# llliuqingyu/RSPL-SLAM

Measured on AMD Instinct MI355X. Metric: stereo frames/sec SuperPoint+SuperGlue+localBA @752x480 (all-keyframe: 2xSP, 2xSG, 1 BA per frame), higher is better.
Workload: dtype fp16 MFMA with fp32 accumulation for SuperPoint/SuperGlue (the reference's TensorRT kFP16 engines), fp32 Sinkhorn/decode, fp64 BA

## Files before the change

rspl-slam_amd/csrc/ba.cpp:

```cpp
#include <immintrin.h>

#include <algorithm>
#include <chrono>
#include <cmath>
#include <cstdlib>
#include <cstring>
#include <limits>
#include <numeric>
#include <string>
#include <type_traits>
#include <memory>
#include <vector>
#include <condition_variable>
#include <deque>
#include <mutex>
#include <thread>

#include "ba_kernels.hpp"
#include "common.hpp"
#include "ba_stage.hpp"
#include "se3_host.hpp"

using namespace rspl;

// ... 364 lines not shown
  Ss = S;
  view_bank(b->bank[1], Ls, Ss);
}

void accept_swap(rspl_ba* b, ba::Problem& P, ba::Lin& Lr, ba::Sys& S, bool lin) {
  std::swap(P.T, P.Tn);
  std::swap(P.X, P.Xn);
  std::swap(P.L, P.Ln);
  if (!lin) return;
  std::swap(b->bank[0], b->bank[1]);
  view_bank(b->bank[0], Lr, S);
}

void arm_prof(rspl_ba* b, const ba::Active& A, ba::Sys& S) {
  if (!b->prof || b->prof_nb[0]) return;
  S.prof = b->prof;
  b->prof_A = A;
  b->prof_nb[0] = ba::chunk_count(A);
  b->prof_nb[1] = ba::update_errors_blocks(A) + A.n_lblk;
  b->prof_nb[2] = ba::update_errors_blocks(A);
  b->prof_nb[3] = A.nchk;
  b->prof_nb[4] = A.K;
}

struct SpecSetup {
  ba::Active A2{};
  uint8_t* level = nullptr;
  int iters2 = 0;
  bool queued = false;
  bool extra = false;
  bool topped_up = false;
};

struct SpecFinish {
  bool on = false;
  ba::Lin L{};
  int E = 0;
  const int* gmap = nullptr;
  uint8_t* inl = nullptr;
  double *Th = nullptr, *Xh = nullptr, *Lh = nullptr;
  unsigned long long q = 0;
};

void preupload_next(rspl_ba* b);

struct DevLmArgs {
  uint8_t* cls_level = nullptr;
  bool build_pp = false;
  SpecFinish* fin = nullptr;
  SpecSetup* nxt = nullptr;
  bool setup_done = false;
};

int optimize_dev(rspl_ba* b, ba::Problem& P, ba::Lin& Lr, ba::Sys& S, const ba::Active& A, int iters,
                 double* chi2_out, int* done_out, const DevLmArgs& d) {
  hipStream_t st = b->stream;
  uint8_t* const cls_level = d.cls_level;
  SpecFinish* const fin = d.fin;
  SpecSetup* const nxt = d.nxt;
  S.lm = b->lmctl;
  S.lm_slot = 0;
  static const bool trace = getenv("RSPL_BA_LMTRACE") != nullptr;
  if (trace && !b->lm_trace) {
    RSPL_HIP(hipMalloc((void**)&b->lm_trace, sizeof(double) * 8 * 64));
    RSPL_HIP(hipMemset(b->lm_trace, 0, sizeof(double) * 8 * 64));
  }
  S.lm_trace = trace ? b->lm_trace + (iters == 10 ? 0 : 8 * 32) : nullptr;
  if (d.setup_done) {
  } else {
    int rg;
    if ((rg = grow_device(b, b->pdg, b->pdg_cap, (size_t)ba::setup_pdg_len(A), (size_t)1 << 14, 4u))) return rg;
    ba::Sys Su = S;
    Su.prof = b->prof && !b->prof_nb[0] && !cls_level ? b->prof : nullptr;
    RSPL_HIP(ba::setup_dev(P, Lr, A, Su, cls_level, cls_level ? const_cast<uint8_t*>(A.lm_act) : nullptr, iters,
                           d.build_pp ? b->pp_cnt : nullptr, b->pp_off, b->pp_buf, b->pdg, st));
  }
  unsigned long long q = b->seq;
  const unsigned long long q_first = b->seq + 1;
  ba::Lin Ls;
  ba::Sys Ss;
  bank_views(b, Lr, S, Ls, Ss);
  int queued = 0;
  const int kev0 = b->kev_used;
  auto enqueue = [&](int n) -> int {
    for (int k = 0; k < n; k++, queued++) {
      q = ++b->seq;
      ba::Spec sp{Ls, Ss};
      if (queued == 3) arm_prof(b, A, S);
      S.lm_slot = queued & 1;
      S.lm_post = k == n - 1;
      hipEvent_t* ev = nullptr;
      if (b->ktime_on) {
        if ((size_t)3 * (b->kev_used + 1) > b->kev.size()) {
          for (int i = 0; i < 3; i++) {
            hipEvent_t e;
            RSPL_HIP(hipEventCreate(&e));
            b->kev.push_back(e);
          }
          b->grew |= 8;
        }
        ev = &b->kev[3 * (size_t)b->kev_used++];
      }
      const hipError_t e = ba::trial_dev(P, Lr, A, S, q, st, sp, ev);
      S.prof = nullptr;
      if (e != hipSuccess) {
        set_error("BA trial launch failed: %s", hipGetErrorString(e));
        return RSPL_E_DEVICE;
      }
    }
    return RSPL_OK;
  };
  int rc;
  unsigned long long q_last = 0;
  auto enqueue_batch = [&](int n) -> int {
    int r;
    if ((r = enqueue(n))) return r;
    q_last = b->seq;
    if (fin) {
      ba::Sys Sf = S;
      Sf.lm = b->lmctl;
      Sf.lm_slot = queued & 1;
      Sf.prof = nullptr;
      fin->q = ++b->seq;
      fin->on = true;
      RSPL_HIP(ba::finish(P, fin->L, fin->E, fin->gmap, fin->inl, fin->Th, fin->Xh, fin->Lh, Sf, fin->q, st));
    }
    return RSPL_OK;
  };
  if ((rc = enqueue_batch(iters))) return rc;
  if (fin) preupload_next(b);
  auto queue_spec_setup = [&]() -> int {
    if (!nxt || (size_t)ba::setup_pdg_len(nxt->A2) > b->pdg_cap) return RSPL_OK;
    ba::Sys S2 = S;
    S2.lm = b->lmctl;
    S2.lm_slot = 0;
    S2.prof = nullptr;
    S2.lm_trace = nullptr;
    RSPL_HIP(ba::setup_dev(P, Lr, nxt->A2, S2, nxt->level, const_cast<uint8_t*>(nxt->A2.lm_act), nxt->iters2,
                           nullptr, b->pp_off, b->pp_buf, b->pdg, st, queued & 1, &Ls, &Ss));
    nxt->queued = true;
    nxt->extra = false;
    return RSPL_OK;
  };
  if ((rc = queue_spec_setup())) return rc;
  double v[4];
  for (;;) {
    if ((rc = spin_mail(b, "the LM trials", [&] {
          const unsigned long long s1 = __atomic_load_n(&b->mail->seq, __ATOMIC_ACQUIRE);
          if (s1 >= q_first && s1 <= q_last) {
            volatile const double* mv = b->mail->v;
            for (int k = 0; k < 4; k++) v[k] = mv[k];
            __atomic_thread_fence(__ATOMIC_ACQUIRE);
            return __atomic_load_n(&b->mail->vseq, __ATOMIC_ACQUIRE) == s1 && (s1 == q_last || v[3] != 0.0);
          }
          if (fin && s1 == fin->q) {
            volatile const double* mv = b->mail->v;
            for (int k = 0; k < 4; k++) v[k] = mv[k];
            __atomic_thread_fence(__ATOMIC_ACQUIRE);
            const unsigned long long vs = __atomic_load_n(&b->mail->vseq, __ATOMIC_ACQUIRE);
            return vs >= q_first && vs <= q_last && v[3] != 0.0;
          }
          return false;
        })))
      return rc;
    if (v[3] != 0.0) {
      if (b->ktime_on) {
        unsigned long long s1 = __atomic_load_n(&b->mail->seq, __ATOMIC_ACQUIRE);
        for (unsigned long long t = q_first; t <= s1 && t <= q_last; t++) b->kev_eval.push_back(kev0 + (int)(t - q_first));
      }
      break;
    }
    if (nxt) nxt->extra = nxt->topped_up = true;
    if ((rc = enqueue_batch(std::max(1, iters - (int)v[1])))) return rc;
    if ((rc = queue_spec_setup())) return rc;
  }
  S.lm = nullptr;
  if (v[2] != 0.0) accept_swap(b, P, Lr, S, true);
  *chi2_out = v[0];
  *done_out = (int)v[1];
  return RSPL_OK;
}

bool dev_lm(const rspl_ba* b, const ba::Active& A, int iters) {
  return b->allreduce == nullptr && iters > 0 && ba::fast_path(A.K);
}

int optimize_host(rspl_ba* b, ba::Problem& P, ba::Lin& Lr, ba::Sys& S, const ba::Active& A, int iters,
                  double* chi2_out, int* done_out) {
  hipStream_t st = b->stream;
  double v[4];
  int rc;
  const bool sh = b->allreduce != nullptr;
  const int n6 = 6 * A.K;
  double* so = b->red + n6 + b->nranks;
  unsigned long long q = ++b->seq;
  RSPL_HIP(ba::compute_errors(P, Lr, A, S, q, st));
  if (sh) {
    if (iters > 0) {
      RSPL_HIP(ba::linearize(P, Lr, A, S, true, st));
      RSPL_HIP(ba::shard_fold(A, S, b->red, b->rank, b->nranks, st));
      if ((rc = allreduce(b, b->red, ba::shard_red_len(A.K, b->nranks)))) return rc;
      RSPL_HIP(ba::shard_post(S, b->red, n6, b->nranks, 0, 0, q, st));
    } else {
      if ((rc = allreduce(b, so, 3))) return rc;
      RSPL_HIP(ba::shard_post(S, b->red, n6, b->nranks, 1, 0, q, st));
    }
  } else if (iters > 0) {
    RSPL_HIP(ba::linearize(P, Lr, A, S, true, st));
    q = ++b->seq;
// ... 699 lines not shown
    A.lmsub = cp.lmsub;
    ba::set_update_geometry(A);
  }
  A.n_line_edges = n_line_local;
  A.ltab = reinterpret_cast<const int4*>(cb + cl.ltab);
  A.n_lblk = n_lblk;
  A.K = K;
  A.nL = nL;
  A.robust = 1;
  A.pp_off = b->pp_off;
  A.pp = b->pp_buf;
  const bool pp_fused = dev_lm(b, A, pr->iterations_first);
  if (!pp_fused) RSPL_HIP(ba::build_pairs(A, b->pp_cnt, b->pp_off, b->pp_buf, st));
  tm.mark("pairs");
  SpecSetup nxt;
  nxt.A2 = A;
  nxt.A2.robust = 0;
  nxt.A2.elevel = level;
  nxt.A2.lm_act = b->lm_act2;
  nxt.level = level;
  nxt.iters2 = pr->iterations_second;
  const bool spec_setup = pp_fused && !sh && !b->ktime_on && dev_lm(b, nxt.A2, pr->iterations_second);
  DevLmArgs d1;
  d1.build_pp = pp_fused;
  d1.nxt = spec_setup ? &nxt : nullptr;
  if ((rc = optimize(b, P, Lr, S, A, pr->iterations_first, &res->chi2_first, &res->iterations_done_first, d1)))
    return rc;
  tm.mark("opt1");
  tr[5] = mono_s();
  uint8_t* inl_h = reinterpret_cast<uint8_t*>(b->stage_dev[c.slot] + dl.inl);
  double* T_h = reinterpret_cast<double*>(b->stage_dev[c.slot] + dl.T);
  double* X_h = reinterpret_cast<double*>(b->stage_dev[c.slot] + dl.X);
  double* L_h = reinterpret_cast<double*>(b->stage_dev[c.slot] + dl.L);
  SpecFinish fin;
  {
    A.robust = 0;
    A.elevel = level;
    A.lm_act = b->lm_act2;
    const bool fused = dev_lm(b, A, pr->iterations_second);
    if (!fused) {
      RSPL_HIP(ba::classify(P, Lr, E, level, nullptr, 0, st));
      RSPL_HIP(ba::landmark_active(A, level, b->lm_act2, st));
    }
    const bool spec_fin = fused && !sh && !b->ktime_on;
    if (spec_fin) {
      fin.L = Lr;
      fin.E = E;
      fin.gmap = reinterpret_cast<const int*>(cb + cl.gmap);
      fin.inl = inl_h;
      fin.Th = T_h;
      fin.Xh = X_h;
      fin.Lh = L_h;
    }
    DevLmArgs d2;
    d2.cls_level = fused ? level : nullptr;
    d2.fin = spec_fin ? &fin : nullptr;
    d2.setup_done = nxt.queued && !nxt.extra;
    if ((rc = optimize(b, P, Lr, S, A, pr->iterations_second, &res->chi2_second, &res->iterations_done_second, d2)))
      return rc;
    tm.mark("opt2");
    tr[6] = mono_s();
    tr[9] = (double)((unsigned)tr[9] | (nxt.queued && !nxt.extra ? 16u : 0u) | (nxt.topped_up ? 32u : 0u));
  }
  const unsigned long long q = fin.on ? fin.q : ++b->seq;
  if (fin.on) {
  } else if (sh) {
    const size_t glen = 3 * (size_t)nq + 6 * (size_t)nl + Eg;
    if ((rc = grow_device(b, b->gbuf, b->gcap, glen, (size_t)1024, 0u))) return rc;
    RSPL_HIP(hipMemsetAsync(b->gbuf, 0, sizeof(double) * glen, st));
    RSPL_HIP(ba::shard_gather(P, Lr, E, reinterpret_cast<const int*>(cb + cl.gmap), b->rank, b->nranks, b->gbuf, st));
    if (glen && (rc = allreduce(b, b->gbuf, glen))) return rc;
    RSPL_HIP(ba::shard_finish(P, Eg, b->gbuf, inl_h, T_h, X_h, L_h, S, q, st));
  } else {
    RSPL_HIP(ba::finish(P, Lr, E, reinterpret_cast<const int*>(cb + cl.gmap), inl_h, T_h, X_h, L_h, S, q, st));
  }
  if ((rc = wait_mail(b, q, nullptr))) return rc;
  if (b->ktime_on) {
    for (int i : b->kev_eval) {
      float a = 0.f, c = 0.f;
      if (hipEventElapsedTime(&a, b->kev[3 * (size_t)i], b->kev[3 * (size_t)i + 1]) == hipSuccess &&
          hipEventElapsedTime(&c, b->kev[3 * (size_t)i + 1], b->kev[3 * (size_t)i + 2]) == hipSuccess) {
        b->kt_ms[0] += a;
        b->kt_ms[1] += c;
        b->kt_n[0]++;
        b->kt_n[1]++;
      }
    }
  }
  if (b->prof && b->prof_nb[0]) report_prof(b);
  tr[9] = (double)((unsigned)tr[9] | b->grew);
  if (b->lm_trace) {
    std::vector<double> h(8 * 64);
    if (hipMemcpy(h.data(), b->lm_trace, sizeof(double) * h.size(), hipMemcpyDeviceToHost) == hipSuccess)
      for (int k = 0; k < 64; k++)
        if (h[8 * k] != 0.0)
          fprintf(stderr, "lmtrace phase %d trial %d chi2 %.17g scale %.6g fail %g lambda %.6g chi0 %.17g cur %g it %g q %g\n",
                  k / 32, k % 32, h[8 * k], h[8 * k + 1], h[8 * k + 2], h[8 * k + 3], h[8 * k + 4], h[8 * k + 5],
                  h[8 * k + 6], h[8 * k + 7]);
    (void)hipMemset(b->lm_trace, 0, sizeof(double) * h.size());
  }
  if (nq) memcpy(res->points, b->stage[c.slot] + dl.X, sizeof(double) * 3 * nq);
  if (nl) memcpy(res->lines, b->stage[c.slot] + dl.L, sizeof(double) * 6 * nl);
  const double* Tout = reinterpret_cast<const double*>(b->stage[c.slot] + dl.T);
  uint8_t* outs[4] = {res->mono_inlier, res->stereo_inlier, res->mono_line_inlier, res->stereo_line_inlier};
  int e = 0;
  for (int t = 0; t < 4; t++) {
    if (outs[t]) memcpy(outs[t], b->stage[c.slot] + dl.inl + e, ne[t]);
    e += ne[t];
  }
// ... 40 lines not shown
```

rspl-slam_amd/csrc/ba_first.hip:

```cpp
#include <hip/hip_runtime.h>

#include <algorithm>
#include <cstdint>

#include "ba_kernels.hpp"
#include "ba_linearize.hpp"

namespace rspl {
namespace ba {

__global__ __launch_bounds__(256) void post_kernel(Sys S, int K, int npd, unsigned long long seq) {
  __shared__ double part[4][64];
  if (npd > 0) {
    const int lane = threadIdx.x & 63, pt = threadIdx.x >> 6, nq6 = 6 * K;
    double mx = 0;
    for (int q0 = 0; q0 < nq6; q0 += 64) {
      const int q = q0 + lane;
      double sacc = 0;
      if (q < nq6) {
        const int pa = q / 6, i = q - 6 * pa;
        const double* src = S.partial2 + (size_t)pa * npd * 6 + i;
        for (int b = pt; b < npd; b += 4) sacc += src[(size_t)b * 6];
      }
      part[pt][lane] = sacc;
// ... 455 lines not shown
  if (g >= A.nL) return;
  uint8_t on = 0;
  for (int k = A.lm_off[g]; k < A.lm_off[g + 1]; k++) on |= level[(k)] == 0;
  lm_act[g] = on;
}

__device__ __forceinline__ bool edge_inlier(const Problem& P, const Lin& L, int e) {
  double chi2;
  bool depth_ok;
  edge_status(P, L, e, chi2, depth_ok);
  return chi2 <= pick4(P.th, P.etype[e]) && depth_ok;
}
__device__ __forceinline__ void classify_edge(const Problem& P, const Lin& L, int e, uint8_t* level, uint8_t* inlier,
                                              int final_pass) {
  if (final_pass) {
    inlier[e] = edge_inlier(P, L, e) ? 1 : 0;
    return;
  }
  double chi2;
  bool depth_ok;
  edge_status(P, L, e, chi2, depth_ok);
  if (chi2 > pick4(P.th, P.etype[e]) || !depth_ok) level[e] = 1;
}

__global__ __launch_bounds__(256) void classify_kernel(Problem P, Lin L, int E, uint8_t* level, uint8_t* inlier,
                                                       int final_pass) {
  const int e = blockIdx.x * blockDim.x + threadIdx.x;
  if (e < E) classify_edge(P, L, e, level, inlier, final_pass);
}

__global__ __launch_bounds__(256) void finish_kernel(Problem P, Lin L, int E, const int* gmap, uint8_t* inl, double* Th,
                                                     double* Xh, double* Lh, Sys S, unsigned long long seq) {
  __shared__ int last;
  if (S.lm) {
    const LmCtrl* c = S.lm + S.lm_slot;
    if (!c->stop) return;
    if (c->cur) bank_state(P);
  }
  const int i = blockIdx.x * blockDim.x + threadIdx.x;
  if (i < E) inl[gmap[i]] = edge_inlier(P, L, i) ? 1 : 0;
  if (i < 8 * P.np) Th[i] = P.T[i];
  if (i < 3 * P.nq) Xh[i] = P.X[i];
  if (i < 6 * P.nl) Lh[i] = P.L[i];
  __threadfence_system();
  __syncthreads();
  if (threadIdx.x == 0) {
    const unsigned tk = __hip_atomic_fetch_add(S.counter, 1u, __ATOMIC_ACQ_REL, __HIP_MEMORY_SCOPE_AGENT);
    last = tk == gridDim.x - 1;
  }
  __syncthreads();
  if (!last || threadIdx.x != 0) return;
  __hip_atomic_store(S.counter, 0u, __ATOMIC_RELAXED, __HIP_MEMORY_SCOPE_AGENT);
  __hip_atomic_store(&S.mail->seq, seq, __ATOMIC_RELEASE, __HIP_MEMORY_SCOPE_SYSTEM);
}

__global__ __launch_bounds__(256) void shard_fold_kernel(Sys S, double* red, int K, int npd, int rank, int nranks) {
  const int n6 = 6 * K;
  for (int q = threadIdx.x; q < n6; q += 256) {
    double acc = 0;
    if (npd > 0) {
      const int pa = q / 6, i = q - 6 * pa;
      const double* src = S.partial2 + (size_t)pa * npd * 6 + i;
      for (int b = 0; b < npd; b++) acc += src[(size_t)b * 6];
    }
    red[q] = acc;
  }
  for (int r = threadIdx.x; r < nranks; r += 256) red[n6 + r] = r == rank ? S.out[2] : 0.0;
}

__global__ void shard_post_kernel(Sys S, const double* red, int n6, int nranks, int mode, int add_pose_scale,
                                  unsigned long long seq) {
// ... 152 lines not shown
```

rspl-slam_amd/csrc/ba_kernels.hpp:

```cpp
#pragma once
#include <hip/hip_runtime.h>

#include <cstdint>

namespace rspl {
namespace ba {

struct Problem {
  const double* cams;
  double* T;
  double* X;
  double* L;
  double* Tn;
  double* Xn;
  double* Ln;
  int np, nq, nl;
  int ncam;
  const int8_t* etype;
  const int* epose;
  const int* elm;
  const int* ecam;
  const double* eobs;
  int Ep;
  double delta[4];
// ... 131 lines not shown
  double* chunk;
  double* pairfin;
  unsigned* pair_ctr;
  unsigned* solve_ctr;
  double* partial;
  double* partial2;
  double* out;
  int* fail;
  unsigned* counter;
  unsigned* lm_ctr;
  Mail* mail;
  double* shard_out;
  int pose_scale;
  unsigned long long* prof;
  LmCtrl* lm;
  double* lm_trace;
  int lm_slot;
  int lm_post;
};
constexpr int kProfPc = 16, kProfUe = kProfPc + 4 * 4096, kProfX = kProfUe + 4 * 4096, kProfLen = kProfX + 8;

constexpr int kLmChunk = 256;
constexpr int kLineBlk = 8;

hipError_t compute_errors(const Problem& P, const Lin& L, const Active& A, Sys& S, unsigned long long seq,
                          hipStream_t s);
hipError_t linearize(const Problem& P, const Lin& L, const Active& A, const Sys& S, bool with_maxdiag,
                     hipStream_t s);
hipError_t post(Sys& S, unsigned long long seq, hipStream_t s, const Active* A = nullptr);
hipError_t setup_dev(const Problem& P, const Lin& L, const Active& A, Sys& S, uint8_t* level, uint8_t* lm_act2,
                     int lm_iters, int* pp_cnt, int* pp_off, int4* pp, double* pdg, hipStream_t s, int gate = -1,
                     const Lin* Ls = nullptr, const Sys* Ss = nullptr);
int setup_pdg_len(const Active& A);
struct Spec {
  Lin Ls;
  Sys Ss;
};
hipError_t trial_host_large(const Problem& P, const Lin& L, const Active& A, Sys& S, double lambda,
                            unsigned long long seq, hipStream_t s);
hipError_t trial_dev(const Problem& P, const Lin& L, const Active& A, Sys& S, unsigned long long seq, hipStream_t s,
                     const Spec& spec, hipEvent_t* ev = nullptr);
hipError_t build_pairs(const Active& A, int* pp_cnt, int* pp_off, int4* pp, hipStream_t s);
hipError_t landmark_active(const Active& A, const uint8_t* level, uint8_t* lm_act, hipStream_t s);
hipError_t classify(const Problem& P, const Lin& L, int E, uint8_t* level, uint8_t* inlier, int final_pass,
                    hipStream_t s);
hipError_t finish(const Problem& P, const Lin& L, int E, const int* gmap, uint8_t* inl, double* Th, double* Xh,
                  double* Lh, Sys& S, unsigned long long seq, hipStream_t s);
hipError_t trial_chunks(const Problem& P, const Lin& L, const Active& A, Sys& S, double lambda, hipStream_t s);
hipError_t trial_solve(const Problem& P, const Lin& L, const Active& A, Sys& S, double lambda, hipStream_t s);
hipError_t shard_fold(const Active& A, Sys& S, double* red, int rank, int nranks, hipStream_t s);
hipError_t shard_post(Sys& S, const double* red, int n6, int nranks, int mode, int add_pose_scale,
                      unsigned long long seq, hipStream_t s);
hipError_t shard_gather(const Problem& P, const Lin& L, int E, const int* gmap, int rank, int nranks, double* G,
                        hipStream_t s);
hipError_t shard_finish(const Problem& P, int E_global, const double* G, uint8_t* inl, double* Th, double* Xh,
                        double* Lh, Sys& S, unsigned long long seq, hipStream_t s);
int shard_red_len(int K, int nranks);
bool fast_path(int K);
bool wave_path(int K);
int update_blocks(const Problem& P);
int errors_blocks(int Ea);
int update_errors_blocks(const Active& A);
void set_update_geometry(Active& A);

}
}
```

rspl-slam_amd/csrc/ba_linearize.hpp:

```cpp
#pragma once
#include "ba_device.hpp"
#include "wave_reduce.hpp"

namespace rspl {
namespace ba {

__device__ __forceinline__ double edge_weight_of(const Problem& P, const Active& A, const double* er, int t) {
  double w = einfo(t);
  if (A.robust) {
    double chi2 = 0;
    for (int k = 0; k < edim(t); k++) chi2 += er[k] * er[k];
    chi2 *= einfo(t);
    double r0, r1;
    huber(chi2, pick4(P.delta, t), r0, r1);
    w *= r1;
  }
  return w;
}

__device__ __forceinline__ void point_jac_R(int t, const double (&R)[9], const double* tt, const double* cam,
                                            const double* Xg, double (&Jp)[3][6], double (&Jl)[3][3]) {
  const double fx = cam[0], fy = cam[1], bf = cam[4];
  double Xc[3];
  mat3_vec(R, Xg, Xc);
// ... 201 lines not shown
    H[8] += lambda;
    const bool ok = small_inv<3>(H, Di);
#pragma unroll
    for (int i = 0; i < 4; i++)
#pragma unroll
      for (int j = 0; j < 4; j++) D[i * 4 + j] = (i < 3 && j < 3) ? Di[i * 3 + j] : 0.0;
    return ok;
  }
  double H[16];
#pragma unroll
  for (int i = 0; i < 16; i++) H[i] = Hll[i];
#pragma unroll
  for (int i = 0; i < 4; i++) H[i * 5] += lambda;
  return small_inv<4>(H, D);
}

__device__ __forceinline__ void cand_pose(const Problem& P, const Active& A, const double* x, int i, bool failed,
                                          double (&o)[8]) {
  const int a = A.pidx[i];
#pragma unroll
  for (int k = 0; k < 8; k++) o[k] = P.T[8 * i + k];
  if (a < 0 || failed) return;
  double xp[6];
#pragma unroll
  for (int k = 0; k < 6; k++) xp[k] = x[6 * a + k];
  const SE3 r = se3_mul(se3_exp(xp), load_T(o));
#pragma unroll
  for (int k = 0; k < 4; k++) o[k] = r.q[k];
#pragma unroll
  for (int k = 0; k < 3; k++) o[4 + k] = r.t[k];
  o[7] = 0;
}

__device__ __forceinline__ void edge_status(const Problem& P, const Lin& L, int e, double& chi2, bool& depth_ok) {
  const int t = P.etype[e];
  chi2 = 0;
  for (int k = 0; k < edim(t); k++) chi2 += L.err[4 * e + k] * L.err[4 * e + k];
  chi2 *= einfo(t);
  depth_ok = true;
  if (t < 2) {
    const SE3 T = load_T(P.T + 8 * P.epose[e]);
    double R[9], Xc[3];
    q_to_R(T.q, R);
    mat3_vec(R, P.X + 3 * P.elm[e], Xc);
    depth_ok = Xc[2] + T.t[2] > 0.0;
  }
}
constexpr int kLinPlain = 0, kLinSpec = 1, kLinSetup = 2;
__device__ __forceinline__ bool edge_outlier(const Problem& P, const Lin& L, int e) {
  double chi2;
  bool depth_ok;
  edge_status(P, L, e, chi2, depth_ok);
  return chi2 > pick4(P.th, P.etype[e]) || !depth_ok;
}
__device__ __forceinline__ bool line_active(const Problem& P, const Lin& L, const Active& A, int g, bool cls) {
  if (!cls) return A.lm_act[g] != 0;
  for (int k = A.lm_off[g]; k < A.lm_off[g + 1]; k++)
    if (!edge_outlier(P, L, k)) return true;
  return false;
}
template <int MODE>
__device__ __forceinline__ void lin_lines(const Problem& P, const Lin& L, const Active& A, const Sys& S, int blk,
                                          bool maxd, const Lin* Lc = nullptr, const Sys* Sc = nullptr,
                                          double lambda = 0.0, bool failed = false,
                                          unsigned long long* stamp = nullptr, bool cls = false,
                                          double* chi_out = nullptr, double* pdg = nullptr, int pd_nb = 0,
                                          int pd_b = 0) {
  constexpr bool SPEC = MODE == kLinSpec, SETUP = MODE == kLinSetup, OWN_ERR = SPEC || SETUP;
  __shared__ double ev[kLineBlk][20][4];
  __shared__ double J[kLineBlk][4 * 6 + 4 * 4];
  __shared__ double Lsh[kLineBlk][6];
  __shared__ double es[kLineBlk][4];
  __shared__ int einfo_s[kLineBlk][4];
  __shared__ double cv[kLineBlk][20];
  __shared__ double Tsh[kLineBlk][8];
  const int tid = threadIdx.x, wv = tid >> 6, lane = tid & 63;
  const int4 tb = A.ltab[blk];
  const int p0 = tb.x, cnt = tb.y & 0xff, gb = tb.z, ge = tb.w;
  const bool split = (tb.y >> 8) != 0;
// ... 354 lines not shown
```

rspl-slam_amd/csrc/ba_trial.hip:

```cpp
#include <hip/hip_runtime.h>

#include <cfloat>
#include <cstdint>

#include "ba_kernels.hpp"
#include "ba_launch.hpp"
#include "ba_linearize.hpp"

namespace rspl {
namespace ba {

__device__ int lm_decide(const LmCtrl* c, LmCtrl* n, double chi2, double scale, double fail) {
  const bool ok = fail == 0.0;
  const double tempChi = ok ? chi2 : DBL_MAX;
  double rho = c->chi - tempChi;
  rho /= ok ? scale + 1e-3 : 1.0;
  double lambda = c->lambda, ni = c->ni;
  int qmax = c->qmax, it = c->it;
  bool brk = false;
  *n = *c;
  if (rho > 0 && isfinite(tempChi) && ok) {
    double alpha = 1. - cube(2 * rho - 1);
    alpha = fmin(alpha, 2. / 3.);
    lambda *= fmax(1. / 3., alpha);
// ... 124 lines not shown
          const double* xp = S.x + 6 * max(as[u], 0);
#pragma unroll
          for (int j = 0; j < 4; j++) {
            double s = 0;
#pragma unroll
            for (int r = 0; r < 6; r++) s += B[r * 4 + j] * xp[r];
            c[j] -= as[u] >= 0 ? s : 0.0;
          }
        }
      }
      double D[16];
      if (!lm_dinv(S.Hll + 16 * g, point, lambda, D)) atomicOr(S.fail, 1);
#pragma unroll
      for (int r = 0; r < 4; r++) xl[r] = D[r * 4] * c[0] + D[r * 4 + 1] * c[1] + D[r * 4 + 2] * c[2] + D[r * 4 + 3] * c[3];
#pragma unroll
      for (int k = 0; k < 4; k++) sc += xl[k] * (lambda * xl[k] + S.bl[4 * g + k]);
    }
    if (point) {
      for (int k = 0; k < 3; k++) P.Xn[3 * g + k] = P.X[3 * g + k] + xl[k];
    } else {
      const int l = g - P.nq;
      double Lv[6];
      for (int k = 0; k < 6; k++) Lv[k] = P.L[6 * l + k];
      if (upd) line_oplus(Lv, xl);
      for (int k = 0; k < 6; k++) P.Ln[6 * l + k] = Lv[k];
    }
  }
  const double s = block_sum256(sc, red);
  if (threadIdx.x == 0) S.partial2[blockIdx.x] = s;
}

template <bool SPEC>
__global__ __launch_bounds__(256) void update_errors_kernel(Problem P, Lin L, Active A, Sys S, double lambda,
                                                            unsigned long long seq, Lin Ls, Sys Ss, int nbu) {
  __shared__ double red[4 * 2];
  __shared__ int last;
  const bool stamp = threadIdx.x == 0 && blockIdx.x < 4096;
  if (stamp) prof_stamp(S, kProfUe + 4 * blockIdx.x);
  bool spec = SPEC;
  if (SPEC && (int)blockIdx.x >= nbu) {
    if (S.lm) {
      LmView v;
      if (!lm_view(S, v)) return;
      lambda = v.lambda;
      spec = v.spec;
      if (v.cur) {
        bank_state(P);
        bank_lin(L, Ls, S, Ss);
      }
    }
    if (!spec) return;
    lin_lines<kLinSpec>(P, Ls, A, Ss, blockIdx.x - nbu, false, &L, &S, lambda, *S.fail != 0,
                    S.prof ? S.prof + kProfUe + 4 * blockIdx.x + 1 : nullptr);
    if (stamp) prof_stamp(S, kProfUe + 4 * blockIdx.x + 3);
    return;
  }
  if (!SPEC) nbu = gridDim.x;
  __shared__ double sT[64 * 8], scam[16 * 5], sx[6 * 32];
  const int tid = threadIdx.x;
  int ub = blockIdx.x;
  if (SPEC && A.ue_bpr > 0) {
    const int b = blockIdx.x, x = b & 7, sl = b >> 3, r = sl / A.ue_bpr, lb = 8 * r + x;
    constexpr int per = 64 * kUeWaves / kGroup;
    ub = lb < A.nchk ? lb * A.ue_bpr + (sl - r * A.ue_bpr) : (A.nL + per - 1) / per + 1;
  }
  const int t = ub * (64 * kUeWaves) + tid, g = t / kGroup, j = t % kGroup;
  const bool in = tid < 64 * kUeWaves && g < A.nL;
  const bool point = g < P.nq;
  int k0 = 0, k1 = 0;
  bool act = false;
  double dl[16], blg[4], lm[6] = {0, 0, 0, 0, 0, 0};
  double dl2[16], blg2[4], lm2[6] = {0, 0, 0, 0, 0, 0};
// ... 7 lines not shown
    act = A.lm_act[g] != 0;
#pragma unroll
    for (int q = 0; q < 16; q++) {
      dl[q] = point && q >= 9 ? 0.0 : S.Hll[16 * g + q];
      dl2[q] = point && q >= 9 ? 0.0 : Ss.Hll[16 * g + q];
    }
#pragma unroll
    for (int q = 0; q < 4; q++) {
      blg[q] = S.bl[4 * g + q];
      blg2[q] = Ss.bl[4 * g + q];
    }
    if (point) {
#pragma unroll
      for (int q = 0; q < 3; q++) {
        lm[q] = P.X[3 * g + q];
        lm2[q] = P.Xn[3 * g + q];
      }
    } else {
#pragma unroll
      for (int q = 0; q < 6; q++) {
        lm[q] = P.L[6 * (g - P.nq) + q];
        lm2[q] = P.Ln[6 * (g - P.nq) + q];
      }
    }
  }
  if (S.lm) {
    LmView v;
    if (!lm_view(S, v)) {
      if (blockIdx.x == 0 && threadIdx.x == 0) S.lm[S.lm_slot ^ 1] = S.lm[S.lm_slot];
      return;
    }
    lambda = v.lambda;
    spec = SPEC && v.spec;
    if (v.cur) {
      bank_state(P);
      bank_lin(L, Ls, S, Ss);
#pragma unroll
      for (int q = 0; q < 16; q++) dl[q] = dl2[q];
#pragma unroll
      for (int q = 0; q < 4; q++) blg[q] = blg2[q];
#pragma unroll
      for (int q = 0; q < 6; q++) lm[q] = lm2[q];
    }
  }
  const bool failed = *S.fail != 0;
  for (int q = tid; q < 5 * P.ncam; q += 256) scam[q] = P.cams[q];
  for (int q = tid; q < 6 * A.K; q += 256) sx[q] = S.x[q];
  const int kf = k0 + j;
  const bool has = in && kf < k1;
  int af = -1, tf = 0, pf = 0, cf = 0, lvf = 0;
  double Bf[24], of[8];
  if (has) {
    af = A.lm_pose[kf];
    tf = P.etype[kf];
    pf = P.epose[kf];
    cf = P.ecam[kf];
    lvf = A.elevel ? A.elevel[kf] : 0;
    load_hpl4(L.Hpl, P.Ep, kf, Bf);
    const double* o = obs_of(P, kf, point ? 0 : 2);
#pragma unroll
    for (int q = 0; q < 8; q++) of[q] = (q < 3 || !point) ? o[q] : 0.0;
  }
  if (tid < P.np) {
    double Tc[8];
    cand_pose(P, A, S.x, tid, failed, Tc);
#pragma unroll
    for (int k = 0; k < 8; k++) sT[8 * tid + k] = Tc[k];
    if (blockIdx.x == 0)
#pragma unroll
      for (int k = 0; k < 8; k++) P.Tn[8 * tid + k] = Tc[k];
  }
  __syncthreads();
  if (stamp) prof_stamp(S, kProfUe + 4 * blockIdx.x + 1);
  const bool upd = in && act && !failed;
  double c[4] = {0, 0, 0, 0};
  if (upd) {
    if (has && af >= 0) {
      const double* xp = sx + 6 * af;
#pragma unroll
      for (int q = 0; q < 4; q++) {
        double s = 0;
#pragma unroll
        for (int r = 0; r < 6; r++) s += Bf[r * 4 + q] * xp[r];
        c[q] -= s;
      }
    }
    for (int k = kf + kGroup; k < k1; k += kGroup) {
      const int a = A.lm_pose[k];
      if (a < 0) continue;
      double B[24];
      load_hpl4(L.Hpl, P.Ep, k, B);
      const double* xp = sx + 6 * a;
#pragma unroll
      for (int q = 0; q < 4; q++) {
        double s = 0;
#pragma unroll
        for (int r = 0; r < 6; r++) s += B[r * 4 + q] * xp[r];
        c[q] -= s;
      }
    }
  }
  group_sum(c);
  double xl[4] = {0, 0, 0, 0};
  double sc = 0, chi = 0;
  if (upd) {
#pragma unroll
    for (int q = 0; q < 4; q++) c[q] += blg[q];
    {
      double D[16];
      if (!lm_dinv(dl, point, lambda, D) && j == 0) atomicOr(S.fail, 1);
#pragma unroll
      for (int q = 0; q < 16; q++) dl[q] = point ? (q < 9 ? D[4 * (q / 3) + q % 3] : 0.0) : D[q];
    }
    if (point) {
#pragma unroll
      for (int r = 0; r < 3; r++) xl[r] = dl[r * 3] * c[0] + dl[r * 3 + 1] * c[1] + dl[r * 3 + 2] * c[2];
    } else {
#pragma unroll
      for (int r = 0; r < 4; r++)
        xl[r] = dl[r * 4] * c[0] + dl[r * 4 + 1] * c[1] + dl[r * 4 + 2] * c[2] + dl[r * 4 + 3] * c[3];
    }
    if (j == 0)
#pragma unroll
      for (int q = 0; q < 4; q++) sc += xl[q] * (lambda * xl[q] + blg[q]);
  }
  const bool lin_pts = SPEC && spec && in && point;
  double hl[9] = {0, 0, 0, 0, 0, 0, 0, 0, 0}, bv[3] = {0, 0, 0};
  if (in) {
    if (point) {
#pragma unroll
      for (int q = 0; q < 3; q++) lm[q] += xl[q];
      if (j == 0)
#pragma unroll
        for (int q = 0; q < 3; q++) P.Xn[3 * g + q] = lm[q];
    } else {
      const int l = g - P.nq;
      if (upd) line_oplus(lm, xl);
      if (j == 0)
#pragma unroll
        for (int q = 0; q < 6; q++) P.Ln[6 * l + q] = lm[q];
    }
    auto edge_cost = [&](int k, int te, int pose, int cam, int lev, const double (&ob)[8], int a) {
      if (lev) {
        if (lin_pts && a >= 0) zero_pose_records<false>(Ls, k);
        return;
      }
      const SE3 T = load_T(sT + 8 * pose);
      const double* cm = scam + 5 * cam;
      double er[4] = {0, 0, 0, 0};
      double chi2;
      if (point) {
        chi2 = point_error(te, cm, ob, T, lm, er);
      } else {
        edge_error(te, cm, ob, T, lm, er);
        chi2 = 0;
#pragma unroll
        for (int q = 0; q < 4; q++)
          if (q < edim(te)) chi2 += er[q] * er[q];
        chi2 *= einfo(te);
      }
#pragma unroll
      for (int q = 0; q < 4; q++) L.err[4 * k + q] = er[q];
      double cst = chi2;
      if (A.robust) {
        double r1;
        huber(chi2, pick4(P.delta, te), cst, r1);
      }
      chi += cst;
      if (lin_pts) point_edge_core<false>(P, Ls, A, k, te, a >= 0, T, cm, lm, er, hl, bv);
    };
    if (has) edge_cost(kf, tf, pf, cf, lvf, of, af);
    for (int k = kf + kGroup; k < k1; k += kGroup) {
      const int te = P.etype[k];
      const double* o = obs_of(P, k, te);
      double ob[8];
#pragma unroll
      for (int q = 0; q < 8; q++) ob[q] = (q < 3 || !point) ? o[q] : 0.0;
      edge_cost(k, te, P.epose[k], P.ecam[k], A.elevel ? A.elevel[k] : 0, ob, A.lm_pose[k]);
    }
  }
  if (SPEC && spec) {
    group_sum(hl);
    group_sum(bv);
    if (in && point && j == 0 && act) {
      double* H = Ss.Hll + 16 * g;
#pragma unroll
      for (int i = 0; i < 9; i++) H[i] = hl[i];
#pragma unroll
      for (int i = 9; i < 16; i++) H[i] = 0.0;
#pragma unroll
      for (int i = 0; i < 3; i++) Ss.bl[4 * g + i] = bv[i];
      Ss.bl[4 * g + 3] = 0.0;
    }
  }
  if (stamp) prof_stamp(S, kProfUe + 4 * blockIdx.x + 2);
  double acc[2] = {chi, sc};
  block_reduce<2>(acc, red);
  if (threadIdx.x == 0) {
    __hip_atomic_store(S.partial + blockIdx.x, red[0], __ATOMIC_RELAXED, __HIP_MEMORY_SCOPE_AGENT);
    __hip_atomic_store(S.partial2 + blockIdx.x, red[1], __ATOMIC_RELAXED, __HIP_MEMORY_SCOPE_AGENT);
    const unsigned tk = ticket(S.counter);
    last = tk == (unsigned)nbu - 1;
  }
  __syncthreads();
  if (stamp) prof_stamp(S, kProfUe + 4 * blockIdx.x + 3);
  if (!last) return;
  double f2[2] = {0, 0};
  for (int k = threadIdx.x; k < nbu; k += 256) {
    f2[0] += __hip_atomic_load(S.partial + k, __ATOMIC_RELAXED, __HIP_MEMORY_SCOPE_AGENT);
    f2[1] += __hip_atomic_load(S.partial2 + k, __ATOMIC_RELAXED, __HIP_MEMORY_SCOPE_AGENT);
  }
  block_reduce<2>(f2, red);
  if (threadIdx.x == 0) {
    const double chi2 = red[0], scale = red[1] + S.out[4];
    const double f = (double)__hip_atomic_load(S.fail, __ATOMIC_RELAXED, __HIP_MEMORY_SCOPE_AGENT);
    const double mx = S.out[2];
    S.out[0] = chi2;
    S.out[1] = scale;
    S.out[3] = f;
    if (S.shard_out) {
      S.shard_out[0] = chi2;
      S.shard_out[1] = red[1];
      S.shard_out[2] = f;
      __hip_atomic_store(S.counter, 0u, __ATOMIC_RELAXED, __HIP_MEMORY_SCOPE_AGENT);
      __hip_atomic_store(S.fail, 0, __ATOMIC_RELAXED, __HIP_MEMORY_SCOPE_AGENT);
      S.out[2] = 0.0;
      return;
    }
    __hip_atomic_store(S.counter, 0u, __ATOMIC_RELAXED, __HIP_MEMORY_SCOPE_AGENT);
    __hip_atomic_store(S.fail, 0, __ATOMIC_RELAXED, __HIP_MEMORY_SCOPE_AGENT);
    S.out[2] = 0.0;
    if (S.lm) {
      LmCtrl* c = S.lm + (S.lm_slot ^ 1);
      const double lam0 = S.lm[S.lm_slot].lambda, chi0 = S.lm[S.lm_slot].chi;
      const int stop = lm_decide(S.lm + S.lm_slot, c, chi2, scale, f);
      if (S.lm_trace && c->trials <= 64) {
        double* t = S.lm_trace + 8 * (c->trials - 1);
        t[0] = chi2; t[1] = scale; t[2] = f; t[3] = lam0; t[4] = chi0; t[5] = c->cur; t[6] = c->it; t[7] = c->qmax;
      }
      if (stop || S.lm_post) post_mail(S.mail, c->chi, (double)c->it, (double)c->cur, (double)stop, seq);
      return;
    }
    post_mail(S.mail, chi2, scale, mx, f, seq);
  }
}

__global__ void shard_fail_stage_kernel(Sys S, double* slot) {
  *slot = (double)__hip_atomic_load(S.fail, __ATOMIC_RELAXED, __HIP_MEMORY_SCOPE_AGENT);
}
__global__ void shard_fail_adopt_kernel(Sys S, const double* slot) {
  __hip_atomic_store(S.fail, *slot != 0.0 ? 1 : 0, __ATOMIC_RELAXED, __HIP_MEMORY_SCOPE_AGENT);
}

int errors_blocks(int Ea) { return Ea > 0 ? (Ea + 255) / 256 : 1; }
int update_blocks(const Problem& P) {
  const int nv = P.np + P.nq + P.nl;
  return nv > 0 ? (nv + 255) / 256 : 1;
}

hipError_t compute_errors(const Problem& P, const Lin& L, const Active& A, Sys& S, unsigned long long seq,
                          hipStream_t s) {
  hipLaunchKernelGGL(errors_kernel, dim3(errors_blocks(A.Ea)), dim3(256), 0, s, P, L, A, S, 0, seq);
  return hipGetLastError();
}

int update_errors_blocks(const Active& A) {
  if (A.ue_bpr > 0) return 8 * ((A.nchk + 7) / 8) * A.ue_bpr;
  return A.nL > 0 ? (A.nL * kGroup + 64 * kUeWaves - 1) / (64 * kUeWaves) : 1;
}

void set_update_geometry(Active& A) {
  constexpr int per = 64 * kUeWaves / kGroup;
  A.ue_bpr = A.nchk >= 8 && A.lmchunk % per == 0 ? A.lmchunk / per : 0;
}

static hipError_t global_tail(const Problem& P, const Lin& L, const Active& A, const Sys& S, double lambda,
                              unsigned long long seq, hipStream_t s) {
  launch_global_solve(A, S, lambda, s);
  const int nbu = update_blocks(P);
  hipLaunchKernelGGL(update_kernel, dim3(nbu), dim3(256), 0, s, P, L, A, S, lambda);
  Problem Pn = P;
  Pn.T = P.Tn; Pn.X = P.Xn; Pn.L = P.Ln;
  hipLaunchKernelGGL(errors_kernel, dim3(errors_blocks(A.Ea)), dim3(256), 0, s, Pn, L, A, S, nbu, seq);
  return hipGetLastError();
}

hipError_t trial_host_large(const Problem& P, const Lin& L, const Active& A, Sys& S, double lambda,
                            unsigned long long seq, hipStream_t s) {
  if (fast_path(A.K)) return hipErrorInvalidValue;
  if (chunk_count(A) > 0) launch_chunks(P, L, A, S, lambda, L, S, false, s);
  return global_tail(P, L, A, S, lambda, seq, s);
}

hipError_t trial_dev(const Problem& P, const Lin& L, const Active& A, Sys& S, unsigned long long seq, hipStream_t s,
                     const Spec& spec, hipEvent_t* ev) {
  if (!S.lm || !fast_path(A.K)) return hipErrorInvalidValue;
  if (ev) (void)hipEventRecord(ev[0], s);
  if (chunk_count(A) > 0) launch_chunks(P, L, A, S, 0.0, spec.Ls, spec.Ss, wave_path(A.K), s);
  const hipError_t e = launch_solve(P, A, S, 0.0, s, true);
  if (e != hipSuccess) return e;
  const int nbu = update_errors_blocks(A), nbl = A.n_lblk;
  if (ev) (void)hipEventRecord(ev[1], s);
  hipLaunchKernelGGL(update_errors_kernel<true>, dim3(nbu + nbl), dim3(256), 0, s, P, L, A, S, 0.0, seq, spec.Ls,
                     spec.Ss, nbu);
  if (ev) (void)hipEventRecord(ev[2], s);
  return hipGetLastError();
}

hipError_t trial_chunks(const Problem& P, const Lin& L, const Active& A, Sys& S, double lambda, hipStream_t s) {
  if (chunk_count(A) > 0) launch_chunks(P, L, A, S, lambda, L, S, false, s);
  hipLaunchKernelGGL(shard_fail_stage_kernel, dim3(1), dim3(1), 0, s, S, S.pairfin + (size_t)A.npairs * 48);
  return hipGetLastError();
}

hipError_t trial_solve(const Problem& P, const Lin& L, const Active& A, Sys& S, double lambda, hipStream_t s) {
  hipLaunchKernelGGL(shard_fail_adopt_kernel, dim3(1), dim3(1), 0, s, S, S.pairfin + (size_t)A.npairs * 48);
  if (!fast_path(A.K)) return global_tail(P, L, A, S, lambda, 0ull, s);
  const hipError_t e = launch_solve(P, A, S, lambda, s, false);
  if (e != hipSuccess) return e;
  hipLaunchKernelGGL(update_errors_kernel<false>, dim3(update_errors_blocks(A)), dim3(256), 0, s, P, L, A, S, lambda,
                     0ull, L, S, 0);
  return hipGetLastError();
}

}
}
```

Before: 1029.

## Fuse BA finish outputs into final LM trial update_errors kernel

Removes the speculative separate finish kernel launch after each LM batch. The last update_errors trial now writes the inlier flags and the staged pose, point and line outputs directly, and signals this through a flag bit in the mailbox. The host then skips the extra finish launch and its mailbox wait when that bit is set. This adds per-edge status computation and extra global writes to the trial kernel. It relies on the fence and waitcnt ordering being correct before the mail is posted.

```diff
diff --git a/rspl-slam_amd/csrc/ba.cpp b/rspl-slam_amd/csrc/ba.cpp
--- a/rspl-slam_amd/csrc/ba.cpp
+++ b/rspl-slam_amd/csrc/ba.cpp
@@ -420,14 +420,9 @@
   bool topped_up = false;
 };
 
-struct SpecFinish {
-  bool on = false;
-  ba::Lin L{};
-  int E = 0;
-  const int* gmap = nullptr;
-  uint8_t* inl = nullptr;
-  double *Th = nullptr, *Xh = nullptr, *Lh = nullptr;
-  unsigned long long q = 0;
+struct FusedFinish {
+  ba::FinOut out{};
+  bool done = false;
 };
 
 void preupload_next(rspl_ba* b);
@@ -435,7 +430,7 @@
 struct DevLmArgs {
   uint8_t* cls_level = nullptr;
   bool build_pp = false;
-  SpecFinish* fin = nullptr;
+  FusedFinish* fin = nullptr;
   SpecSetup* nxt = nullptr;
   bool setup_done = false;
 };
@@ -444,7 +439,7 @@
                  double* chi2_out, int* done_out, const DevLmArgs& d) {
   hipStream_t st = b->stream;
   uint8_t* const cls_level = d.cls_level;
-  SpecFinish* const fin = d.fin;
+  FusedFinish* const fin = d.fin;
   SpecSetup* const nxt = d.nxt;
   S.lm = b->lmctl;
   S.lm_slot = 0;
@@ -470,10 +465,12 @@
   bank_views(b, Lr, S, Ls, Ss);
   int queued = 0;
   const int kev0 = b->kev_used;
+  unsigned long long q_last = 0;
   auto enqueue = [&](int n) -> int {
     for (int k = 0; k < n; k++, queued++) {
       q = ++b->seq;
       ba::Spec sp{Ls, Ss};
+      if (fin) sp.fin = fin->out;
       if (queued == 3) arm_prof(b, A, S);
       S.lm_slot = queued & 1;
       S.lm_post = k == n - 1;
@@ -496,26 +493,11 @@
         return RSPL_E_DEVICE;
       }
     }
+    q_last = b->seq;
     return RSPL_OK;
   };
   int rc;
-  unsigned long long q_last = 0;
-  auto enqueue_batch = [&](int n) -> int {
-    int r;
-    if ((r = enqueue(n))) return r;
-    q_last = b->seq;
-    if (fin) {
-      ba::Sys Sf = S;
-      Sf.lm = b->lmctl;
-      Sf.lm_slot = queued & 1;
-      Sf.prof = nullptr;
-      fin->q = ++b->seq;
-      fin->on = true;
-      RSPL_HIP(ba::finish(P, fin->L, fin->E, fin->gmap, fin->inl, fin->Th, fin->Xh, fin->Lh, Sf, fin->q, st));
-    }
-    return RSPL_OK;
-  };
-  if ((rc = enqueue_batch(iters))) return rc;
+  if ((rc = enqueue(iters))) return rc;
   if (fin) preupload_next(b);
   auto queue_spec_setup = [&]() -> int {
     if (!nxt || (size_t)ba::setup_pdg_len(nxt->A2) > b->pdg_cap) return RSPL_OK;
@@ -541,13 +523,6 @@
             __atomic_thread_fence(__ATOMIC_ACQUIRE);
             return __atomic_load_n(&b->mail->vseq, __ATOMIC_ACQUIRE) == s1 && (s1 == q_last || v[3] != 0.0);
           }
-          if (fin && s1 == fin->q) {
-            volatile const double* mv = b->mail->v;
-            for (int k = 0; k < 4; k++) v[k] = mv[k];
-            __atomic_thread_fence(__ATOMIC_ACQUIRE);
-            const unsigned long long vs = __atomic_load_n(&b->mail->vseq, __ATOMIC_ACQUIRE);
-            return vs >= q_first && vs <= q_last && v[3] != 0.0;
-          }
           return false;
         })))
       return rc;
@@ -559,10 +534,11 @@
       break;
     }
     if (nxt) nxt->extra = nxt->topped_up = true;
-    if ((rc = enqueue_batch(std::max(1, iters - (int)v[1])))) return rc;
+    if ((rc = enqueue(std::max(1, iters - (int)v[1])))) return rc;
     if ((rc = queue_spec_setup())) return rc;
   }
   S.lm = nullptr;
+  if (fin) fin->done = ((int)v[3] & 2) != 0;
   if (v[2] != 0.0) accept_swap(b, P, Lr, S, true);
   *chi2_out = v[0];
   *done_out = (int)v[1];
@@ -1328,7 +1304,7 @@
   double* T_h = reinterpret_cast<double*>(b->stage_dev[c.slot] + dl.T);
   double* X_h = reinterpret_cast<double*>(b->stage_dev[c.slot] + dl.X);
   double* L_h = reinterpret_cast<double*>(b->stage_dev[c.slot] + dl.L);
-  SpecFinish fin;
+  FusedFinish fin;
   {
     A.robust = 0;
     A.elevel = level;
@@ -1338,28 +1314,21 @@
       RSPL_HIP(ba::classify(P, Lr, E, level, nullptr, 0, st));
       RSPL_HIP(ba::landmark_active(A, level, b->lm_act2, st));
     }
-    const bool spec_fin = fused && !sh && !b->ktime_on;
-    if (spec_fin) {
-      fin.L = Lr;
-      fin.E = E;
-      fin.gmap = reinterpret_cast<const int*>(cb + cl.gmap);
-      fin.inl = inl_h;
-      fin.Th = T_h;
-      fin.Xh = X_h;
-      fin.Lh = L_h;
-    }
+    const bool fuse_fin = fused && !sh && !b->ktime_on;
+    if (fuse_fin) fin.out = ba::FinOut{reinterpret_cast<const int*>(cb + cl.gmap), inl_h, T_h, X_h, L_h};
     DevLmArgs d2;
     d2.cls_level = fused ? level : nullptr;
-    d2.fin = spec_fin ? &fin : nullptr;
+    d2.fin = fuse_fin ? &fin : nullptr;
     d2.setup_done = nxt.queued && !nxt.extra;
     if ((rc = optimize(b, P, Lr, S, A, pr->iterations_second, &res->chi2_second, &res->iterations_done_second, d2)))
       return rc;
     tm.mark("opt2");
     tr[6] = mono_s();
-    tr[9] = (double)((unsigned)tr[9] | (nxt.queued && !nxt.extra ? 16u : 0u) | (nxt.topped_up ? 32u : 0u));
-  }
-  const unsigned long long q = fin.on ? fin.q : ++b->seq;
-  if (fin.on) {
+    tr[9] = (double)((unsigned)tr[9] | (nxt.queued && !nxt.extra ? 16u : 0u) | (nxt.topped_up ? 32u : 0u) |
+                     (fin.done ? 64u : 0u));
+  }
+  const unsigned long long q = fin.done ? 0 : ++b->seq;
+  if (fin.done) {
   } else if (sh) {
     const size_t glen = 3 * (size_t)nq + 6 * (size_t)nl + Eg;
     if ((rc = grow_device(b, b->gbuf, b->gcap, glen, (size_t)1024, 0u))) return rc;
@@ -1370,7 +1339,7 @@
   } else {
     RSPL_HIP(ba::finish(P, Lr, E, reinterpret_cast<const int*>(cb + cl.gmap), inl_h, T_h, X_h, L_h, S, q, st));
   }
-  if ((rc = wait_mail(b, q, nullptr))) return rc;
+  if (!fin.done && (rc = wait_mail(b, q, nullptr))) return rc;
   if (b->ktime_on) {
     for (int i : b->kev_eval) {
       float a = 0.f, c = 0.f;
diff --git a/rspl-slam_amd/csrc/ba_first.hip b/rspl-slam_amd/csrc/ba_first.hip
--- a/rspl-slam_amd/csrc/ba_first.hip
+++ b/rspl-slam_amd/csrc/ba_first.hip
@@ -511,11 +511,6 @@
 __global__ __launch_bounds__(256) void finish_kernel(Problem P, Lin L, int E, const int* gmap, uint8_t* inl, double* Th,
                                                      double* Xh, double* Lh, Sys S, unsigned long long seq) {
   __shared__ int last;
-  if (S.lm) {
-    const LmCtrl* c = S.lm + S.lm_slot;
-    if (!c->stop) return;
-    if (c->cur) bank_state(P);
-  }
   const int i = blockIdx.x * blockDim.x + threadIdx.x;
   if (i < E) inl[gmap[i]] = edge_inlier(P, L, i) ? 1 : 0;
   if (i < 8 * P.np) Th[i] = P.T[i];
diff --git a/rspl-slam_amd/csrc/ba_kernels.hpp b/rspl-slam_amd/csrc/ba_kernels.hpp
--- a/rspl-slam_amd/csrc/ba_kernels.hpp
+++ b/rspl-slam_amd/csrc/ba_kernels.hpp
@@ -187,9 +187,15 @@
                      int lm_iters, int* pp_cnt, int* pp_off, int4* pp, double* pdg, hipStream_t s, int gate = -1,
                      const Lin* Ls = nullptr, const Sys* Ss = nullptr);
 int setup_pdg_len(const Active& A);
+struct FinOut {
+  const int* gmap = nullptr;
+  uint8_t* inl = nullptr;
+  double *Th = nullptr, *Xh = nullptr, *Lh = nullptr;
+};
 struct Spec {
   Lin Ls;
   Sys Ss;
+  FinOut fin{};
 };
 hipError_t trial_host_large(const Problem& P, const Lin& L, const Active& A, Sys& S, double lambda,
                             unsigned long long seq, hipStream_t s);
diff --git a/rspl-slam_amd/csrc/ba_linearize.hpp b/rspl-slam_amd/csrc/ba_linearize.hpp
--- a/rspl-slam_amd/csrc/ba_linearize.hpp
+++ b/rspl-slam_amd/csrc/ba_linearize.hpp
@@ -257,19 +257,24 @@
   o[7] = 0;
 }
 
-__device__ __forceinline__ void edge_status(const Problem& P, const Lin& L, int e, double& chi2, bool& depth_ok) {
-  const int t = P.etype[e];
+__device__ __forceinline__ void edge_status_at(int t, const double* err, const double* Tp, const double* X,
+                                               double& chi2, bool& depth_ok) {
   chi2 = 0;
-  for (int k = 0; k < edim(t); k++) chi2 += L.err[4 * e + k] * L.err[4 * e + k];
+#pragma unroll
+  for (int k = 0; k < 4; k++)
+    if (k < edim(t)) chi2 += err[k] * err[k];
   chi2 *= einfo(t);
   depth_ok = true;
   if (t < 2) {
-    const SE3 T = load_T(P.T + 8 * P.epose[e]);
+    const SE3 T = load_T(Tp);
     double R[9], Xc[3];
     q_to_R(T.q, R);
-    mat3_vec(R, P.X + 3 * P.elm[e], Xc);
+    mat3_vec(R, X, Xc);
     depth_ok = Xc[2] + T.t[2] > 0.0;
   }
+}
+__device__ __forceinline__ void edge_status(const Problem& P, const Lin& L, int e, double& chi2, bool& depth_ok) {
+  edge_status_at(P.etype[e], L.err + 4 * e, P.T + 8 * P.epose[e], P.X + 3 * P.elm[e], chi2, depth_ok);
 }
 constexpr int kLinPlain = 0, kLinSpec = 1, kLinSetup = 2;
 __device__ __forceinline__ bool edge_outlier(const Problem& P, const Lin& L, int e) {
diff --git a/rspl-slam_amd/csrc/ba_trial.hip b/rspl-slam_amd/csrc/ba_trial.hip
--- a/rspl-slam_amd/csrc/ba_trial.hip
+++ b/rspl-slam_amd/csrc/ba_trial.hip
@@ -180,12 +180,14 @@
 
 template <bool SPEC>
 __global__ __launch_bounds__(256) void update_errors_kernel(Problem P, Lin L, Active A, Sys S, double lambda,
-                                                            unsigned long long seq, Lin Ls, Sys Ss, int nbu) {
+                                                            unsigned long long seq, Lin Ls, Sys Ss, int nbu,
+                                                            FinOut F) {
   __shared__ double red[4 * 2];
   __shared__ int last;
   const bool stamp = threadIdx.x == 0 && blockIdx.x < 4096;
   if (stamp) prof_stamp(S, kProfUe + 4 * blockIdx.x);
   bool spec = SPEC;
+  bool finw = false;
   if (SPEC && (int)blockIdx.x >= nbu) {
     if (S.lm) {
       LmView v;
@@ -259,6 +261,7 @@
     }
     lambda = v.lambda;
     spec = SPEC && v.spec;
+    finw = SPEC && F.inl != nullptr && !v.spec;
     if (v.cur) {
       bank_state(P);
       bank_lin(L, Ls, S, Ss);
@@ -293,9 +296,13 @@
     cand_pose(P, A, S.x, tid, failed, Tc);
 #pragma unroll
     for (int k = 0; k < 8; k++) sT[8 * tid + k] = Tc[k];
-    if (blockIdx.x == 0)
+    if (blockIdx.x == 0) {
 #pragma unroll
       for (int k = 0; k < 8; k++) P.Tn[8 * tid + k] = Tc[k];
+      if (finw)
+#pragma unroll
+        for (int k = 0; k < 8; k++) F.Th[8 * tid + k] = Tc[k];
+    }
   }
   __syncthreads();
   if (stamp) prof_stamp(S, kProfUe + 4 * blockIdx.x + 1);
@@ -357,19 +364,34 @@
     if (point) {
 #pragma unroll
       for (int q = 0; q < 3; q++) lm[q] += xl[q];
-      if (j == 0)
+      if (j == 0) {
 #pragma unroll
         for (int q = 0; q < 3; q++) P.Xn[3 * g + q] = lm[q];
+        if (finw)
+#pragma unroll
+          for (int q = 0; q < 3; q++) F.Xh[3 * g + q] = lm[q];
+      }
     } else {
       const int l = g - P.nq;
       if (upd) line_oplus(lm, xl);
-      if (j == 0)
+      if (j == 0) {
 #pragma unroll
         for (int q = 0; q < 6; q++) P.Ln[6 * l + q] = lm[q];
-    }
+        if (finw)
+#pragma unroll
+          for (int q = 0; q < 6; q++) F.Lh[6 * l + q] = lm[q];
+      }
+    }
+    auto flag = [&](int k, int te, int pose, const double* err) {
+      double chi2;
+      bool depth_ok;
+      edge_status_at(te, err, sT + 8 * pose, lm, chi2, depth_ok);
+      F.inl[F.gmap[k]] = chi2 <= pick4(P.th, te) && depth_ok ? 1 : 0;
+    };
     auto edge_cost = [&](int k, int te, int pose, int cam, int lev, const double (&ob)[8], int a) {
       if (lev) {
         if (lin_pts && a >= 0) zero_pose_records<false>(Ls, k);
+        if (finw) flag(k, te, pose, L.err + 4 * k);
         return;
       }
       const SE3 T = load_T(sT + 8 * pose);
@@ -395,6 +417,7 @@
       }
       chi += cst;
       if (lin_pts) point_edge_core<false>(P, Ls, A, k, te, a >= 0, T, cm, lm, er, hl, bv);
+      if (finw) flag(k, te, pose, er);
     };
     if (has) edge_cost(kf, tf, pf, cf, lvf, of, af);
     for (int k = kf + kGroup; k < k1; k += kGroup) {
@@ -421,9 +444,11 @@
     }
   }
   if (stamp) prof_stamp(S, kProfUe + 4 * blockIdx.x + 2);
+  if (finw) asm volatile("s_waitcnt vmcnt(0)" ::: "memory");
   double acc[2] = {chi, sc};
   block_reduce<2>(acc, red);
   if (threadIdx.x == 0) {
+    if (finw) __builtin_amdgcn_fence(__ATOMIC_RELEASE, "");
     __hip_atomic_store(S.partial + blockIdx.x, red[0], __ATOMIC_RELAXED, __HIP_MEMORY_SCOPE_AGENT);
     __hip_atomic_store(S.partial2 + blockIdx.x, red[1], __ATOMIC_RELAXED, __HIP_MEMORY_SCOPE_AGENT);
     const unsigned tk = ticket(S.counter);
@@ -465,7 +490,8 @@
         double* t = S.lm_trace + 8 * (c->trials - 1);
         t[0] = chi2; t[1] = scale; t[2] = f; t[3] = lam0; t[4] = chi0; t[5] = c->cur; t[6] = c->it; t[7] = c->qmax;
       }
-      if (stop || S.lm_post) post_mail(S.mail, c->chi, (double)c->it, (double)c->cur, (double)stop, seq);
+      const int fused = finw && stop && c->cur != S.lm[S.lm_slot].cur ? 2 : 0;
+      if (stop || S.lm_post) post_mail(S.mail, c->chi, (double)c->it, (double)c->cur, (double)(stop | fused), seq);
       return;
     }
     post_mail(S.mail, chi2, scale, mx, f, seq);
@@ -529,7 +555,7 @@
   const int nbu = update_errors_blocks(A), nbl = A.n_lblk;
   if (ev) (void)hipEventRecord(ev[1], s);
   hipLaunchKernelGGL(update_errors_kernel<true>, dim3(nbu + nbl), dim3(256), 0, s, P, L, A, S, 0.0, seq, spec.Ls,
-                     spec.Ss, nbu);
+                     spec.Ss, nbu, spec.fin);
   if (ev) (void)hipEventRecord(ev[2], s);
   return hipGetLastError();
 }
@@ -546,7 +572,7 @@
   const hipError_t e = launch_solve(P, A, S, lambda, s, false);
   if (e != hipSuccess) return e;
   hipLaunchKernelGGL(update_errors_kernel<false>, dim3(update_errors_blocks(A)), dim3(256), 0, s, P, L, A, S, lambda,
-                     0ull, L, S, 0);
+                     0ull, L, S, 0, FinOut{});
   return hipGetLastError();
 }
 
```

Result: no change. 1048 (median of 3 runs) (+1.8%).
